# danieleschmidt/spin-torque-rl-gym

Measured on AMD Instinct MI355X. Metric: env_steps_per_sec, higher is better.
Workload: dtype f64

## Files before the change

### spin-torque-rl-gym_amd/csrc/stg_physics.hpp

```cpp
#pragma once

#include <hip/hip_runtime.h>
#include <stdint.h>
#include <type_traits>

#include "stg_minstep.hpp"

namespace stg {

enum ClassConst : int {
    C_EX = 0, C_EY, C_EZ,
    C_HK,
    C_MS,
    C_ALPHA,
    C_GEFF,
    C_POL,
    C_MSV,
    C_HS_SIMPLE,
    C_RX, C_RY, C_RZ,
    C_DX, C_DY, C_DZ,
    C_HEX,
    C_BETA, C_BETAP,
    C_GAMMA,
    C_HS_LLGS,
    C_KUV,
    C_EDEMAG,
    C_NX, C_NY, C_NZ,
    C_AREA, C_RP, C_RAP, C_TMR,
    C_REFX, C_REFY, C_REFZ,
    C_RSERIES,
    C_DEVTYPE,
    C_VALID,
    C_SOT_DL, C_SOT_FL,
    C_SIGX, C_SIGY, C_SIGZ,
    C_KU,
    C_VCMA_XI, C_VCMA_TD2,
    C_VCMA_VBD,
    C_MU0MS,
    C_COUNT
};

template <class P>
__host__ __device__ inline void derive_row(const P& p, double gamma, double temperature, double* r) {
#pragma clang fp contract(off)
    const double mu0 = 4 * 3.14159265358979323846 * 1e-7;
    const double en = sqrt((p.easy_axis[0] * p.easy_axis[0] + p.easy_axis[1] * p.easy_axis[1]) + p.easy_axis[2] * p.easy_axis[2]);
    r[C_EX] = p.easy_axis[0] / en; r[C_EY] = p.easy_axis[1] / en; r[C_EZ] = p.easy_axis[2] / en;
    r[C_HK] = (2 * p.ku) / (mu0 * p.ms);
    r[C_MS] = p.ms;
    r[C_ALPHA] = p.damping;
    r[C_GEFF] = gamma / (1 + p.damping * p.damping);
    r[C_POL] = p.polarization;
    r[C_MSV] = p.ms * p.volume;
    r[C_HS_SIMPLE] = sqrt(2 * p.damping * 1.38e-23 * temperature / (mu0 * p.ms * p.volume * gamma));
    r[C_RX] = p.easy_axis[0]; r[C_RY] = p.easy_axis[1]; r[C_RZ] = p.easy_axis[2];
    r[C_DX] = -p.ms * p.demag[0]; r[C_DY] = -p.ms * p.demag[1]; r[C_DZ] = -p.ms * p.demag[2];
    r[C_HEX] = p.a_ex > 0 ? (2 * p.a_ex / (mu0 * p.ms)) * 0.1 : 0.0;
    r[C_BETA] = p.polarization * gamma / (2 * p.ms * p.volume);
    r[C_BETAP] = 0.1 * r[C_BETA];
    r[C_GAMMA] = gamma;
    r[C_HS_LLGS] = sqrt(2 * p.damping * 1.380649e-23 * temperature / (gamma * mu0 * p.ms * p.volume));
    r[C_KUV] = p.ku * p.volume;
    r[C_EDEMAG] = 0.5 * mu0 * (p.ms * p.ms) * p.volume;
    r[C_NX] = p.demag[0]; r[C_NY] = p.demag[1]; r[C_NZ] = p.demag[2];
    r[C_AREA] = p.area; r[C_RP] = p.r_p; r[C_RAP] = p.r_ap;
    r[C_TMR] = (p.r_ap - p.r_p) / p.r_p;
    const double rn = sqrt((p.ref_m[0] * p.ref_m[0] + p.ref_m[1] * p.ref_m[1]) + p.ref_m[2] * p.ref_m[2]);
    r[C_REFX] = p.ref_m[0] / rn; r[C_REFY] = p.ref_m[1] / rn; r[C_REFZ] = p.ref_m[2] / rn;
    r[C_RSERIES] = p.r_series;
    r[C_DEVTYPE] = (double)p.dev_type;
    r[C_VALID] = p.params_valid ? 1.0 : 0.0;
    r[C_SOT_DL] = p.sot_tau_dl; r[C_SOT_FL] = p.sot_tau_fl;
    r[C_SIGX] = p.sot_sigma[0]; r[C_SIGY] = p.sot_sigma[1]; r[C_SIGZ] = p.sot_sigma[2];
    r[C_KU] = p.ku;
    r[C_VCMA_XI] = p.vcma_xi;
    r[C_VCMA_TD2] = p.vcma_td * p.vcma_td;
    r[C_VCMA_VBD] = p.vcma_vbd;
    r[C_MU0MS] = mu0 * p.ms;
}

struct V3 {
    double x, y, z;
};

__device__ __forceinline__ double mul_x(double a, double b) {
#pragma clang fp contract(off)
    const double r = a * b;
    return r;
}
__device__ __forceinline__ double add_x(double a, double b) {
#pragma clang fp contract(off)
    const double r = a + b;
    return r;
}
__device__ __forceinline__ double sub_x(double a, double b) {
#pragma clang fp contract(off)
    const double r = a - b;
    return r;
}

__device__ __forceinline__ double rsqrt_fast(double s) {
    const double y = __builtin_amdgcn_rsq(s);
    const double e = __builtin_fma(-(s * y), y, 1.0);
    return __builtin_fma(y * e, __builtin_fma(0.375, e, 0.5), y);
}

__device__ __forceinline__ void batch_ready(double at, double a0, double a1, double a2, double b0, double b1, double b2) {
    asm volatile("" : : "v"(at), "v"(a0), "v"(a1), "v"(a2), "v"(b0), "v"(b1), "v"(b2));
}

__device__ __forceinline__ double vgpr_const(double c) {
    asm volatile("" : "+v"(c));
    return c;
}

__device__ __forceinline__ double fmax_abs(double a, double b) {
    double r;
    asm("v_max_f64 %0, |%1|, |%2|" : "=v"(r) : "v"(a), "v"(b));
    return r;
}

__device__ __forceinline__ void commit_step(unsigned long long mask, double& d0, double s0, double& d1, double s1, double& d2, double s2,
                                            double& d3, double s3, double& d4, double s4, double& d5, double s5, double& d6, double s6) {
    unsigned long long saved;
    asm("s_and_saveexec_b64 %[sv], %[m]\n\t"
        "v_mov_b64 %[d0], %[s0]\n\t"
        "v_mov_b64 %[d1], %[s1]\n\t"
        "v_mov_b64 %[d2], %[s2]\n\t"
        "v_mov_b64 %[d3], %[s3]\n\t"
        "v_mov_b64 %[d4], %[s4]\n\t"
        "v_mov_b64 %[d5], %[s5]\n\t"
        "v_mov_b64 %[d6], %[s6]\n\t"
        "s_mov_b64 exec, %[sv]"
        : [d0] "+v"(d0), [d1] "+v"(d1), [d2] "+v"(d2), [d3] "+v"(d3), [d4] "+v"(d4), [d5] "+v"(d5), [d6] "+v"(d6), [sv] "=&s"(saved)
        : [s0] "v"(s0), [s1] "v"(s1), [s2] "v"(s2), [s3] "v"(s3), [s4] "v"(s4), [s5] "v"(s5), [s6] "v"(s6), [m] "s"(mask)
        : "scc");
}

__device__ __forceinline__ double rcp_fast(double x) {
    const double y = __builtin_amdgcn_rcp(x);
    return __builtin_fma(y, __builtin_fma(-x, y, 1.0), y);
}

__device__ __forceinline__ double inv_tenth_root(double e2, double tenth = 0.1) {
    const double y = (double)__builtin_amdgcn_exp2f(-0.1f * __builtin_amdgcn_logf((float)e2));
    const double y2 = y * y, y4 = y2 * y2, y8 = y4 * y4;
    const double e = __builtin_fma(-e2, y8 * y2, 1.0);
    return __builtin_fma(y * e, __builtin_fma(0.055, e, tenth), y);
}

__device__ __forceinline__ double fifth_root(double x) {
    int e;
    const double mant = frexp(x, &e);
    const double t = -0.2 * ((double)e + (double)__builtin_amdgcn_logf((float)mant));
    const double ti = rint(t);
    double r = ldexp((double)__builtin_amdgcn_exp2f((float)(t - ti)), (int)ti);
    const double r2 = r * r, r4 = r2 * r2;
    const double err = __builtin_fma(-x, r4 * r, 1.0);
    r = __builtin_fma(r * err, __builtin_fma(0.12, err, 0.2), r);
    const double q2 = r * r;
    return x * (q2 * q2);
}

__device__ __forceinline__ V3 cross(const V3& a, const V3& b) {
#pragma clang fp contract(off)
    return V3{__builtin_fma(a.y, b.z, -(a.z * b.y)), __builtin_fma(a.z, b.x, -(a.x * b.z)), __builtin_fma(a.x, b.y, -(a.y * b.x))};
}
__device__ __forceinline__ double dot(const V3& a, const V3& b) {
#pragma clang fp contract(off)
    return __builtin_fma(a.z, b.z, __builtin_fma(a.y, b.y, a.x * b.x));
}
__device__ __forceinline__ V3 scale3(double c, const V3& z) {
#pragma clang fp contract(off)
    return V3{c * z.x, c * z.y, c * z.z};
}
__device__ __forceinline__ bool finite3(const V3& a) { return isfinite(a.x) && isfinite(a.y) && isfinite(a.z); }

__device__ __forceinline__ void philox4x32_10(uint32_t c0, uint32_t c1, uint32_t c2, uint32_t c3, uint32_t k0,
                                              uint32_t k1, uint32_t (&out)[4]) {
#pragma unroll
    for (int r = 0; r < 10; ++r) {
        const uint32_t hi0 = __umulhi(0xD2511F53u, c0), lo0 = 0xD2511F53u * c0;
        const uint32_t hi1 = __umulhi(0xCD9E8D57u, c2), lo1 = 0xCD9E8D57u * c2;
        const uint32_t n0 = hi1 ^ c1 ^ k0, n2 = hi0 ^ c3 ^ k1;
        c0 = n0; c1 = lo1; c2 = n2; c3 = lo0;
        k0 += 0x9E3779B9u; k1 += 0xBB67AE85u;
    }
    out[0] = c0; out[1] = c1; out[2] = c2; out[3] = c3;
}

struct NormalStream {
    uint32_t s0, s1, s2, s3;
    float carry;
    __device__ __forceinline__ void init(uint64_t seed, uint64_t env_id, uint32_t env_step, uint32_t tag) {
        uint32_t r[4];
        philox4x32_10((uint32_t)env_id, (uint32_t)(env_id >> 32), env_step, tag, (uint32_t)seed, (uint32_t)(seed >> 32), r);
        s0 = r[0]; s1 = r[1]; s2 = r[2]; s3 = r[3] | 1u;
        carry = 0.0f;
    }
    __device__ __forceinline__ uint32_t next() {
        const uint32_t result = s0 + s3;
        const uint32_t t = s1 << 9;
        s2 ^= s0; s3 ^= s1; s1 ^= s2; s0 ^= s3; s2 ^= t;
        s3 = (s3 << 11) | (s3 >> 21);
        return result;
    }
    __device__ __forceinline__ float uniform() {
        return __uint_as_float(__builtin_amdgcn_alignbit(0x7fu, next(), 9u)) - 0.99999994f;
    }
    typedef float f32x2 __attribute__((ext_vector_type(2)));
    __device__ __forceinline__ void pair(float& a, float& b) {
        float t, c, s_;
        pair_head(t, c, s_);
        finish_pair(t, c, s_, a, b);
    }
    __device__ __forceinline__ void pair_head(float& t, float& c, float& s_) {
        f32x2 u{__uint_as_float(__builtin_amdgcn_alignbit(0x7fu, next(), 9u)), __uint_as_float(__builtin_amdgcn_alignbit(0x7fu, next(), 9u))};
        u = u - f32x2{0.99999994f, 0.99999994f};
        t = -1.3862943611198906f * __builtin_amdgcn_logf(u.x);
        c = __builtin_amdgcn_cosf(u.y);
        s_ = __builtin_amdgcn_sinf(u.y);
    }
    static __device__ __forceinline__ void finish_pair(float t, float c, float s_, float& a, float& b) {
        const float r = __builtin_amdgcn_sqrtf(t);
        const f32x2 cs = f32x2{c, s_} * f32x2{r, r};
        a = cs.x;
        b = cs.y;
    }
    __device__ __forceinline__ V3 draw3_even() {
        float a, b, c, d;
        pair(a, b);
        pair(c, d);
        carry = d;
        return V3{(double)a, (double)b, (double)c};
    }
    __device__ __forceinline__ V3 draw3_odd() {
        float a, b;
        pair(a, b);
        return V3{(double)carry, (double)a, (double)b};
    }
};

struct RngKey {
    uint64_t seed, env_id;
    uint32_t env_step;
};

struct InlineNormals {
    static constexpr bool kShared = false, kScaled = false;
    NormalStream ns;
    __device__ __forceinline__ void begin(const RngKey& rk) { ns.init(rk.seed, rk.env_id, rk.env_step, 0u); }
    __device__ __forceinline__ V3 draw(bool even) { return even ? ns.draw3_even() : ns.draw3_odd(); }
    static constexpr bool broken = false;
    __device__ __forceinline__ void peek() {}
    __device__ __forceinline__ bool chunk_end(bool lane_continues) { return lane_continues; }
    __device__ __forceinline__ bool chunk_end_wave(bool mine) { return mine; }
    __device__ __forceinline__ int32_t chunk_end_go(int32_t go) { return go; }
};

constexpr int SHARED_SUBS_RK4 = 2;
constexpr int SHARED_SUBS3 = 4 * SHARED_SUBS_RK4;
constexpr int SHARED_CHUNK_FIXED = 12 * SHARED_SUBS_RK4;
constexpr int SHARED_CHUNK_RK45 = 18;
constexpr int PC_STOP = 1 << 30;
constexpr int PC_SPIN_CAP = 1 << 22;

typedef __attribute__((address_space(3))) int lds_int;
__device__ __forceinline__ volatile lds_int* lds_flag(const int* p) { return (volatile lds_int*)p; }

template <int WGW>
__device__ __forceinline__ bool any_flag(volatile lds_int* f) {
    int v = f[0];
#pragma unroll
    for (int j = 1; j < WGW; ++j) v |= f[j];
    return v != 0;
}
__device__ __forceinline__ int pc_load(const int* p) {
    return __builtin_amdgcn_readfirstlane(__hip_atomic_load(p, __ATOMIC_ACQUIRE, __HIP_MEMORY_SCOPE_WORKGROUP));
}
__device__ __forceinline__ void pc_store(int* p, int v) {
    __hip_atomic_store(p, v, __ATOMIC_RELEASE, __HIP_MEMORY_SCOPE_WORKGROUP);
}

template <typename T, bool SCALED, int DEPTH, bool BARRIER>
struct SharedNormalsT {
    static constexpr int CHUNK = SCALED ? SHARED_CHUNK_RK45 : SHARED_CHUNK_FIXED;
    static_assert(!BARRIER || DEPTH == 2, "the barrier form runs the producer exactly one chunk ahead");
    static constexpr bool kShared = true, kScaled = SCALED;
    const T* buf;
    int* hs;
    int lane, it, idx, seen;
    bool broken;
    static constexpr bool kToggle = BARRIER && SCALED;
    int slot_b, flag_b;
    __device__ __forceinline__ void begin(const RngKey&) {
        it = 0; idx = 0; seen = 1; broken = false;
        if (kToggle) {
            static_assert(((CHUNK * 64) & 63) == 0, "the slot bit and the lane bits are disjoint");
            slot_b = lane * (int)sizeof(T); flag_b = 0;
            asm volatile("" : "+v"(slot_b), "+v"(flag_b));
        }
    }
    __device__ __forceinline__ V3 draw(bool) {
        const T* b = kToggle ? (const T*)((const char*)buf + slot_b) + idx * 64 : buf + ((it & (DEPTH - 1)) * CHUNK + idx) * 64 + lane;
        idx += 3;
        return V3{(double)b[0], (double)b[64], (double)b[128]};
    }
    __device__ __forceinline__ void peek() {
        if (!BARRIER) seen = __hip_atomic_load(hs, __ATOMIC_RELAXED, __HIP_MEMORY_SCOPE_WORKGROUP);
    }
    __device__ __forceinline__ bool chunk_end(bool lane_continues) { return chunk_end_wave(__ballot(lane_continues) != 0ull); }
    __device__ __forceinline__ bool chunk_end_wave(bool mine) { return chunk_end_go(mine ? 1 : 0) != 0; }
    __device__ __forceinline__ int32_t chunk_end_go(int32_t go) {
        const bool mine = go != 0;
        if (BARRIER) {
            if (kToggle) {
                *(volatile lds_int*)((volatile __attribute__((address_space(3))) char*)lds_flag(hs) + flag_b) = go;
                flag_b ^= (int)sizeof(int); slot_b ^= CHUNK * 64 * (int)sizeof(T);
            } else {
                lds_flag(hs)[it & 1] = go;
            }
            __syncthreads();
            ++it;
            idx = 0;
            return go;
        }
        ++it;
        idx = 0;
        pc_store(hs + 1, it | (mine ? 0 : PC_STOP));
        int have = __builtin_amdgcn_readfirstlane(seen);
        if (__builtin_expect(mine && have <= it, 0)) {
            int spins = 0;
#pragma unroll 1
            do {
                if (spins) __builtin_amdgcn_s_sleep(1);
                have = pc_load(hs);
            } while (have <= it && ++spins <= PC_SPIN_CAP);
            broken = broken || have <= it;
        }
        seen = have;
        __builtin_amdgcn_fence(__ATOMIC_ACQUIRE, "workgroup");
        return (mine && !broken) ? 1 : 0;
    }
};

template <typename T, bool SCALED, int DEPTH, bool BARRIER>
__device__ __forceinline__ void produce_normals(T* buf, int* hs, int lane, const RngKey& rk, int n_first, int n_chunk, double c) {
    NormalStream ns;
    ns.init(rk.seed, rk.env_id, rk.env_step, 0u);
    bool even = true;
    auto fill = [&](int slot, int count) {
        T* b = buf + (slot * (SCALED ? SHARED_CHUNK_RK45 : SHARED_CHUNK_FIXED)) * 64 + lane;
        for (int j = 0; j < count; j += 3) {
            V3 z = even ? ns.draw3_even() : ns.draw3_odd();
            if (SCALED) z = scale3(c, z);
            even = !even;
            b[(j + 0) * 64] = (T)z.x; b[(j + 1) * 64] = (T)z.y; b[(j + 2) * 64] = (T)z.z;
        }
    };
    fill(0, n_first);
    if (!BARRIER) pc_store(hs, 1);
    __syncthreads();
    if (BARRIER) {
        for (int k = 1;; ++k) {
            fill(k & 1, n_chunk);
            __syncthreads();
            if (lds_flag(hs)[(k - 1) & 1] == 0) return;
        }
    }
    for (int k = 1;; ++k) {
        int v = pc_load(hs + 1);
#pragma unroll 1
        for (int spins = 0; (v & (PC_STOP - 1)) < k - DEPTH + 1 && !(v & PC_STOP); ++spins) {
            if (spins > PC_SPIN_CAP) return;
            __builtin_amdgcn_s_sleep(1);
            v = pc_load(hs + 1);
        }
        if (v & PC_STOP) return;
        fill(k & (DEPTH - 1), n_chunk);
        pc_store(hs, k + 1);
    }
}

struct SimpleK {
    V3 e;
    double ghk;
    double gdm;
    double alpha;
    double ghs;
};
__device__ __forceinline__ SimpleK make_simple(const V3& e, double hk, double ms, double alpha, double geff, double hs) {
#pragma clang fp contract(off)
    return SimpleK{e, -geff * hk, geff * ms, alpha, -geff * hs};
}
struct LlgsK {
    V3 r;
    V3 gd;
    double ghk, ghex;
    double alpha;
    double ghs;
    double gz;
    double agz;
};
__device__ __forceinline__ LlgsK make_llgs(const V3& r, const V3& d, double hk, double hex, double alpha, double gamma, double hs) {
#pragma clang fp contract(off)
    const double ng = -gamma;
    const double gz = ng * ((hk * r.z) * r.z + d.z);
    return LlgsK{r, V3{ng * d.x, ng * d.y, ng * d.z}, ng * hk, ng * hex, alpha, ng * hs, gz, alpha * gz};
}


template <bool THERMAL, bool AXIS_Z>
__device__ __forceinline__ V3 simple_rhs(const V3& m, const SimpleK& k, double ghk, double aJ, const V3& z) {
#pragma clang fp contract(off)
    if (AXIS_Z) {
        const double gz = (ghk + k.gdm) * m.z;
        V3 p;
        if (THERMAL) {
            const V3 g{k.ghs * z.x, k.ghs * z.y, __builtin_fma(k.ghs, z.z, gz)};
            p = cross(m, g);
        } else {
            p = V3{m.y * gz, -(m.x * gz), 0.0};
        }
        const double wx = __builtin_fma(k.alpha, p.x, aJ * m.y), wy = __builtin_fma(k.alpha, p.y, -(aJ * m.x));
        if (THERMAL) {
            const double wz = k.alpha * p.z;
            return V3{__builtin_fma(m.y, wz, __builtin_fma(-m.z, wy, p.x)), __builtin_fma(m.z, wx, __builtin_fma(-m.x, wz, p.y)),
                      __builtin_fma(m.x, wy, __builtin_fma(-m.y, wx, p.z))};
        }
        return V3{__builtin_fma(-m.z, wy, p.x), __builtin_fma(m.z, wx, p.y), __builtin_fma(m.x, wy, -(m.y * wx))};
    }
    const V3 t = cross(m, k.e);
    const double c = ghk * dot(m, k.e);
    const double d = k.gdm * m.z;
    V3 p;
    if (THERMAL) {
        const V3 g{__builtin_fma(k.ghs, z.x, c * k.e.x), __builtin_fma(k.ghs, z.y, c * k.e.y),
                   __builtin_fma(k.ghs, z.z, __builtin_fma(c, k.e.z, d))};
        p = cross(m, g);
    } else {
        p = V3{__builtin_fma(c, t.x, d * m.y), __builtin_fma(c, t.y, -(d * m.x)), c * t.z};
    }
    const V3 w{__builtin_fma(k.alpha, p.x, aJ * t.x), __builtin_fma(k.alpha, p.y, aJ * t.y),
               __builtin_fma(k.alpha, p.z, aJ * t.z)};
    return V3{__builtin_fma(m.y, w.z, __builtin_fma(-m.z, w.y, p.x)), __builtin_fma(m.z, w.x, __builtin_fma(-m.x, w.z, p.y)),
              __builtin_fma(m.x, w.y, __builtin_fma(-m.y, w.x, p.z))};
}

struct DevTorque {
    double sdl, sfl;
    V3 sigma;
    double ghk_pulse;
    bool any_sot;
};

__device__ __forceinline__ double vcma_keff(double volt, double ku, double xi, double td2, double vbd) {
    const double v = volt < -vbd ? -vbd : (volt > vbd ? vbd : volt);
    const double keff = ku + (-xi * fabs(v) / td2);
    return fmax(keff, -0.5 * ku);
}

template <bool THERMAL, bool AXIS_Z, bool DEVPHYS>
__device__ __forceinline__ V3 simple_stage(const V3& m, const SimpleK& k, double aJ, const V3& z, const DevTorque& dv,
                                           bool on) {
#pragma clang fp contract(off)
    if (!DEVPHYS) return simple_rhs<THERMAL, AXIS_Z>(m, k, k.ghk, aJ, z);
    V3 f = simple_rhs<THERMAL, AXIS_Z>(m, k, on ? dv.ghk_pulse : k.ghk, aJ, z);
    if (dv.any_sot) {
        const double a = on ? dv.sdl : 0.0, b = on ? dv.sfl : 0.0;
        const V3 sxm = cross(dv.sigma, m);
        f = V3{f.x + __builtin_fma(a, sxm.x, b * dv.sigma.x), f.y + __builtin_fma(a, sxm.y, b * dv.sigma.y),
               f.z + __builtin_fma(a, sxm.z, b * dv.sigma.z)};
    }
    return f;
}

__device__ __forceinline__ int simple_validate(V3& m, bool& zero_row) {
#pragma clang fp contract(off)
    zero_row = false;
    const double e = __builtin_fma(m.z, m.z, __builtin_fma(m.y, m.y, __builtin_fma(m.x, m.x, -1.0)));
    const bool near1 = fabs(e) < 0.0009765625;
    const double inv1 = __builtin_fma(e, __builtin_fma(e, __builtin_fma(e, __builtin_fma(e, 0.2734375, -0.3125), 0.375), -0.5), 1.0);
    if (__builtin_expect(__ballot(!near1) == 0ull, 1)) {
        m = V3{m.x * inv1, m.y * inv1, m.z * inv1};
        return 0;
    }
    const double s = dot(m, m);
    const double inv = near1 ? inv1 : rsqrt_fast(s);
    const bool ordinary = (s >= 1e-24) && (s <= 1.7976931348623157e308);
    if (__builtin_expect(__ballot(!ordinary) == 0ull, 1)) {
        m = V3{m.x * inv, m.y * inv, m.z * inv};
        return 0;
    }
    if (!finite3(m) || s < 1e-24) { m = V3{0.0, 0.0, 1.0}; return 1; }
    m = V3{m.x * inv, m.y * inv, m.z * inv};
    zero_row = isinf(s);
    return 0;
}

__device__ __forceinline__ bool validation_rejects(const V3& m) {
    return !finite3(m) || sqrt(dot(m, m)) < 1e-12;
}

struct SolveOut {
    V3 m;
    int32_t n;
    int32_t resets;
    int64_t work;
    bool ok;
};

struct Recorder {
    double* t;
    double* m;
    double* e;
    double* tq;
    int64_t N, i;
    int32_t cap;
    __device__ __forceinline__ void put(int32_t row, double tt, const V3& mm, double ee, double tqv = 0.0) const {
        if (row < cap) {
            if (t) t[(int64_t)row * N + i] = tt;
            if (m) {
                double* b = m + (int64_t)row * 3 * N + i;
                b[0] = mm.x; b[N] = mm.y; b[2 * N] = mm.z;
            }
            if (e) e[(int64_t)row * N + i] = ee;
            if (tq) tq[(int64_t)row * N + i] = tqv;
        }
    }
};

template <int METHOD, bool THERMAL, bool RECORD, bool AXIS_Z, bool DEVPHYS, class NSRC>
__device__ __forceinline__ SolveOut simple_solve(const V3& m0, double J, double T, const SimpleK& k, double pol,
                                                 double msv, bool class_valid, double temperature, double max_step,
                                                 const RngKey& rk, const Recorder& rec, const DevTorque& dv, NSRC& ns,
                                                 double inv_tau, bool enabled) {
#pragma clang fp contract(off)
    SolveOut o{m0, 0, 0, 0, false};
    const bool rejected_in = !enabled || validation_rejects(m0) || !(T > 0.0) || !class_valid || !(temperature > 0.0);
    if (!NSRC::kShared && rejected_in) return o;
    V3 m = m0;
    bool zr;
    int resets = simple_validate(m, zr);
    double dt = fmin(max_step, (T / 100.0));
    int n = (int)(T / dt);
    n = n < 10 ? 10 : n;
    dt = T / (double)n;
    if (NSRC::kShared && rejected_in) n = 0;
    o.n = n;
    o.work = n;
    const double half_dt = 0.5 * dt, sixth_dt = dt / 6.0;
    const bool useJ = fabs(J) > 1e-12;
    const double aJ = useJ ? (pol * J) / msv : 0.0;
    const double kJ = aJ;
    const double t_last = mul_x((double)(n - 1), dt);
    const bool on2_last = add_x(t_last, mul_x(dt, 0.5)) <= T, on4_last = add_x(t_last, dt) <= T;
    const double kJ2_last = on2_last ? kJ : 0.0;
    const double kJ4_last = on4_last ? kJ : 0.0;
    bool fail = false;
    const V3 zero{0.0, 0.0, 0.0};
    if (THERMAL) ns.begin(rk);
    const bool ou_sel = THERMAL && inv_tau > 0.0;
    double ou_d = 0.0, ou_c = 1.0;
    V3 ou_x = zero;
    if (ou_sel) {
        ou_d = exp(-dt * inv_tau);
        ou_c = sqrt(1.0 - ou_d * ou_d);
    }
    if (RECORD) rec.put(0, 0.0, m, 0.0);
    auto run = [&](auto ou_tag) {
    constexpr bool ou = decltype(ou_tag)::value;
    auto substep = [&](int i, auto which_tag) {
        constexpr int WHICH = decltype(which_tag)::value;
        const bool last = WHICH == 2 ? (i == n - 1) : (WHICH == 1);
        const double kJ2 = last ? kJ2_last : kJ, kJ4 = last ? kJ4_last : kJ;
        const bool on2 = !last || on2_last, on4 = !last || on4_last;
        V3 mn;
        if (METHOD == 1) {
            V3 z0 = zero;
            if (THERMAL) z0 = ns.draw((i & 1) == 0);
            if (ou) {
                ou_x = V3{__builtin_fma(ou_d, ou_x.x, ou_c * z0.x), __builtin_fma(ou_d, ou_x.y, ou_c * z0.y),
                          __builtin_fma(ou_d, ou_x.z, ou_c * z0.z)};
                z0 = ou_x;
            }
            const V3 f = simple_stage<THERMAL, AXIS_Z, DEVPHYS>(m, k, kJ, z0, dv, true);
            mn = V3{__builtin_fma(dt, f.x, m.x), __builtin_fma(dt, f.y, m.y), __builtin_fma(dt, f.z, m.z)};
        } else {
            V3 z0 = zero, z1 = zero, z2 = zero, z3 = zero;
            if (ou) {
                const V3 xi = ns.draw((i & 1) == 0);
                ou_x = V3{__builtin_fma(ou_d, ou_x.x, ou_c * xi.x), __builtin_fma(ou_d, ou_x.y, ou_c * xi.y),
                          __builtin_fma(ou_d, ou_x.z, ou_c * xi.z)};
                z0 = ou_x; z1 = ou_x; z2 = ou_x; z3 = ou_x;
            } else if (THERMAL) {
                z0 = ns.draw(true); z1 = ns.draw(false); z2 = ns.draw(true); z3 = ns.draw(false);
            }
            const V3 f1 = simple_stage<THERMAL, AXIS_Z, DEVPHYS>(m, k, kJ, z0, dv, true);
            const V3 y2{__builtin_fma(half_dt, f1.x, m.x), __builtin_fma(half_dt, f1.y, m.y), __builtin_fma(half_dt, f1.z, m.z)};
            const V3 f2 = simple_stage<THERMAL, AXIS_Z, DEVPHYS>(y2, k, kJ2, z1, dv, on2);
            const V3 y3{__builtin_fma(half_dt, f2.x, m.x), __builtin_fma(half_dt, f2.y, m.y), __builtin_fma(half_dt, f2.z, m.z)};
            const V3 f3 = simple_stage<THERMAL, AXIS_Z, DEVPHYS>(y3, k, kJ2, z2, dv, on2);
            if (THERMAL) ns.peek();
            const V3 y4{__builtin_fma(dt, f3.x, m.x), __builtin_fma(dt, f3.y, m.y), __builtin_fma(dt, f3.z, m.z)};
            const V3 f4 = simple_stage<THERMAL, AXIS_Z, DEVPHYS>(y4, k, kJ4, z3, dv, on4);
            mn = V3{__builtin_fma(sixth_dt, __builtin_fma(2.0, f2.x, f1.x) + __builtin_fma(2.0, f3.x, f4.x), m.x),
                    __builtin_fma(sixth_dt, __builtin_fma(2.0, f2.y, f1.y) + __builtin_fma(2.0, f3.y, f4.y), m.y),
                    __builtin_fma(sixth_dt, __builtin_fma(2.0, f2.z, f1.z) + __builtin_fma(2.0, f3.z, f4.z), m.z)};
        }
        resets += simple_validate(mn, zr);
        fail |= zr;
        m = mn;
        if (RECORD) rec.put(i + 1, last ? T : mul_x((double)(i + 1), dt), m, 0.0);
    };
    if (NSRC::kShared) {
        constexpr int SUBS = (METHOD == 1 || ou) ? SHARED_SUBS3 : SHARED_SUBS_RK4;
        for (int i = 0;; ++i) {
            if (i < n) substep(i, std::integral_constant<int, 2>{});
            if (SUBS == 1 || (i & (SUBS - 1)) == SUBS - 1) {
                if (!ns.chunk_end(i + 1 < n)) break;
            }
        }
    } else {
        for (int i = 0; i < n - 1; ++i) substep(i, std::integral_constant<int, 0>{});
        substep(n - 1, std::integral_constant<int, 1>{});
    }
    };
    if (THERMAL && ou_sel) run(std::true_type{}); else run(std::false_type{});
    const bool rejected_shared = NSRC::kShared && rejected_in;
    o.resets = rejected_shared ? 0 : resets;
    if (fail || rejected_shared || ns.broken) return o;
    o.m = m;
    o.ok = true;
    return o;
}

template <bool THERMAL, bool AXIS_Z, bool CHECKED = true>
__device__ __forceinline__ V3 llgs_rhs(const V3& y, const LlgsK& k, double bJ, double bpJ, const V3& ht) {
#pragma clang fp contract(off)
    const double ss = dot(y, y);
    const double inv = rsqrt_fast(ss);
    V3 m{y.x * inv, y.y * inv, y.z * inv};
    if (CHECKED) {
        const bool unit = ss > 1e-24;
        if (__builtin_expect(__ballot(!unit) != 0ull, 0)) m = V3{unit ? m.x : 0.0, unit ? m.y : 0.0, unit ? m.z : 1.0};
    }
    if (AXIS_Z) {
        const double u = __builtin_fma(k.gz, m.z, bpJ);
        const double w = __builtin_fma(k.agz, m.z, bJ);
        if (!THERMAL) {
            const double c = m.z * w;
            return V3{__builtin_fma(m.x, c, m.y * u), __builtin_fma(m.y, c, -(m.x * u)), __builtin_fma(m.z, c, -w)};
        }
        const double uz = ht.z + u;
        const V3 W{k.alpha * ht.x, k.alpha * ht.y, __builtin_fma(k.alpha, ht.z, w)};
        const double s = dot(m, W);
        return V3{__builtin_fma(m.x, s, __builtin_fma(m.y, uz, __builtin_fma(-m.z, ht.y, -W.x))),
                  __builtin_fma(m.y, s, __builtin_fma(m.z, ht.x, __builtin_fma(-m.x, uz, -W.y))),
                  __builtin_fma(m.z, s, __builtin_fma(m.x, ht.y, __builtin_fma(-m.y, ht.x, -W.z)))};
    }
    const double c = k.ghk * dot(m, k.r);
    V3 g{(c * k.r.x + k.gd.x * m.x) + k.ghex * m.x, (c * k.r.y + k.gd.y * m.y) + k.ghex * m.y,
         (c * k.r.z + k.gd.z * m.z) + k.ghex * m.z};
    if (THERMAL) g = V3{g.x + ht.x, g.y + ht.y, g.z + ht.z};
    const V3 U{g.x, g.y, g.z + bpJ};
    const V3 W{k.alpha * g.x, k.alpha * g.y, __builtin_fma(k.alpha, g.z, bJ)};
    const double s = dot(m, W);
    return V3{__builtin_fma(m.x, s, __builtin_fma(m.y, U.z, __builtin_fma(-m.z, U.y, -W.x))),
              __builtin_fma(m.y, s, __builtin_fma(m.z, U.x, __builtin_fma(-m.x, U.z, -W.y))),
              __builtin_fma(m.z, s, __builtin_fma(m.x, U.y, __builtin_fma(-m.y, U.x, -W.z)))};
}

struct LlgsEnergyK {
    double kuv, edemag;
    V3 r, nfac;
};
__device__ __forceinline__ double llgs_energy(const V3& m, const LlgsEnergyK& k) {
    const double ct = dot(m, k.r);
    return -k.kuv * (ct * ct) + k.edemag * (k.nfac.x * (m.x * m.x) + k.nfac.y * (m.y * m.y) + k.nfac.z * (m.z * m.z));
}

__device__ __forceinline__ double llgs_torque_norms(const V3& m, double bJ, double bpJ) {
#pragma clang fp contract(off)
    const V3 mxp{m.y, -m.x, 0.0};
    const V3 mm = cross(m, mxp);
    const V3 a{bJ * mm.x, bJ * mm.y, bJ * mm.z}, b{bpJ * mxp.x, bpJ * mxp.y, bpJ * mxp.z};
    return sqrt((a.x * a.x + a.y * a.y) + a.z * a.z) + sqrt((b.x * b.x + b.y * b.y) + b.z * b.z);
}

__device__ __forceinline__ double rms3(const V3& a) { return sqrt(dot(a, a)) / 1.7320508075688772; }

struct Dp5Tab {
    double A51, A52, A53, A54, A61, A62, A63, A64, A65, E1, E3, E4, E5, E6, E7;
    double B4, third, c09, tenth;
};
__device__ __forceinline__ Dp5Tab make_dp5_tab() {
    Dp5Tab t;
    t.A51 = vgpr_const(19372.0 / 6561); t.A52 = vgpr_const(-25360.0 / 2187); t.A53 = vgpr_const(64448.0 / 6561); t.A54 = vgpr_const(-212.0 / 729);
    t.A61 = vgpr_const(9017.0 / 3168); t.A62 = vgpr_const(-355.0 / 33); t.A63 = vgpr_const(46732.0 / 5247); t.A64 = vgpr_const(49.0 / 176);
    t.A65 = vgpr_const(-5103.0 / 18656);
    t.E1 = vgpr_const(-71.0 / 57600); t.E3 = vgpr_const(71.0 / 16695); t.E4 = vgpr_const(-71.0 / 1920); t.E5 = vgpr_const(17253.0 / 339200);
    t.E6 = vgpr_const(-22.0 / 525); t.E7 = vgpr_const(1.0 / 40);
    t.B4 = vgpr_const(125.0 / 192); t.third = vgpr_const(1.0 / 3.0); t.c09 = vgpr_const(0.9); t.tenth = vgpr_const(0.1);
    return t;
}

struct LlgsLane {
    V3 y, f;
    V3 m0;
    double t, T, h_abs;
    double h_floor;
    double bJ, bpJ;
    int32_t attempts;
    int32_t npts;
    bool idle;
    bool rejected, active;
};

typedef unsigned long long lanemask;
struct LlgsMasks {
    lanemask active, pacc, low;
};
__device__ __forceinline__ bool lane_in(lanemask m) { return __builtin_amdgcn_inverse_ballot_w64(m); }
__device__ __forceinline__ LlgsMasks llgs_masks_open(const LlgsLane& L) {
    return LlgsMasks{__ballot(L.active), __ballot(!L.rejected), __ballot(L.h_abs < L.h_floor)};
}
__device__ __forceinline__ void llgs_masks_close(LlgsLane& L, const LlgsMasks& M) {
    L.active = lane_in(M.active);
    L.rejected = !lane_in(M.pacc);
}

template <bool RECORD>
__device__ __forceinline__ void llgs_lane_emit(LlgsLane& L, V3& out_m, const Recorder& rec, const LlgsEnergyK& ek) {
    const double inv = rsqrt_fast(dot(L.y, L.y));
    out_m = V3{L.y.x * inv, L.y.y * inv, L.y.z * inv};
    if (RECORD) rec.put(L.npts, L.t, out_m, rec.e ? llgs_energy(out_m, ek) : 0.0, rec.tq ? llgs_torque_norms(out_m, L.bJ, L.bpJ) : 0.0);
    ++L.npts;
}

template <bool THERMAL, bool AXIS_Z, bool CHECKED = true>
__device__ __forceinline__ V3 llgs_fun(const LlgsLane& L, const LlgsK& k, const V3& y, const V3& ht, bool on) {
    return llgs_rhs<THERMAL, AXIS_Z, CHECKED>(y, k, on ? L.bJ : 0.0, on ? L.bpJ : 0.0, ht);
}
template <bool THERMAL, class NSRC>
__device__ __forceinline__ V3 llgs_draw(NSRC& ns, const LlgsK& k, bool even) {
    if (!THERMAL) return V3{0.0, 0.0, 0.0};
    return NSRC::kScaled ? ns.draw(even) : scale3(k.ghs, ns.draw(even));
}

template <bool THERMAL, bool RECORD, bool AXIS_Z, class NSRC>
__device__ __forceinline__ void llgs_lane_begin(LlgsLane& L, V3& out_m, const V3& m0, double J, double T, const LlgsK& k, double beta,
                                                double betap, double rtol, double atol, double max_step, const RngKey& rk,
                                                const Recorder& rec, const LlgsEnergyK& ek, NSRC& ns, bool enabled) {
    const bool useJ = !(fabs(J) < 1e-12);
    L.bJ = useJ ? beta * J : 0.0;
    L.bpJ = useJ ? betap * J : 0.0;
    L.m0 = m0;
    L.T = T;
    if (THERMAL) ns.begin(rk);
    const double n0 = rsqrt_fast(dot(m0, m0));
    L.y = V3{m0.x * n0, m0.y * n0, m0.z * n0};
    L.t = 0.0;
    L.npts = 0;
    if (RECORD) llgs_lane_emit<RECORD>(L, out_m, rec, ek); else ++L.npts;
    L.f = llgs_fun<THERMAL, AXIS_Z>(L, k, L.y, llgs_draw<THERMAL>(ns, k, true), true);
    double h_abs;
    {
        const V3& y = L.y;
        const V3& f = L.f;
        const V3 sc{atol + fabs(y.x) * rtol, atol + fabs(y.y) * rtol, atol + fabs(y.z) * rtol};
        const V3 isc{rcp_fast(sc.x), rcp_fast(sc.y), rcp_fast(sc.z)};
        const double d0 = rms3(V3{y.x * isc.x, y.y * isc.y, y.z * isc.z});
        const double d1 = rms3(V3{f.x * isc.x, f.y * isc.y, f.z * isc.z});
        double h0 = (d0 < 1e-5 || d1 < 1e-5) ? 1e-6 : (0.01 * d0) * rcp_fast(d1);
        h0 = fmin(h0, T);
        const V3 y1{y.x + h0 * f.x, y.y + h0 * f.y, y.z + h0 * f.z};
        const V3 f1 = llgs_fun<THERMAL, AXIS_Z>(L, k, y1, llgs_draw<THERMAL>(ns, k, false), true);
        const double d2 = rms3(V3{(f1.x - f.x) * isc.x, (f1.y - f.y) * isc.y, (f1.z - f.z) * isc.z}) * rcp_fast(h0);
        const double h1 = (d1 <= 1e-15 && d2 <= 1e-15) ? fmax(1e-6, h0 * 1e-3) : fifth_root(0.01 * rcp_fast(fmax(d1, d2)));
        h_abs = fmin(fmin(100.0 * h0, h1), fmin(T, max_step));
    }
    L.rejected = false;
    L.attempts = 0;
    const double min_step = min_step_at(L.t);
    L.h_abs = h_abs > max_step ? max_step : (h_abs < min_step ? min_step : h_abs);
    L.h_floor = isfinite(T) ? min_step_at(T) : __builtin_inf();
    L.active = enabled && (L.t != T);
    L.idle = !L.active;
}

template <bool UNIFORM_IT>
__device__ __forceinline__ void llgs_lane_gate(LlgsLane& L, LlgsMasks& M, int32_t max_attempts) {
    if (__builtin_expect((M.low & M.active) != 0ull, 0)) {
        const double min_step = min_step_at(L.t);
        if (lane_in(M.pacc)) L.h_abs = L.h_abs < min_step ? min_step : L.h_abs;
        M.active &= ~__ballot(L.h_abs < min_step);
    }
    if (!UNIFORM_IT) M.active &= ~__ballot(L.attempts >= max_attempts);
}

__device__ __forceinline__ int32_t attempt_loop_next(lanemask& active, lanemask not_arrived, int32_t& it, int32_t budget) {
    int32_t go;
    asm("s_add_i32 %[it], %[it], 1\n\t"
        "s_and_b64 %[act], %[act], %[na]\n\t"
        "s_cselect_b32 %[go], %[bud], 0\n\t"
        "s_cmp_lt_i32 %[it], %[go]\n\t"
        "s_cselect_b32 %[go], 1, 0"
        : [act] "+s"(active), [it] "+s"(it), [go] "=&s"(go)
        : [na] "s"(not_arrived), [bud] "s"(budget)
        : "scc");
    return go;
}

template <bool THERMAL, bool RECORD, bool AXIS_Z, bool UNIFORM_IT, class NSRC>
__device__ __forceinline__ void llgs_lane_attempt(LlgsLane& L, LlgsMasks& M, V3& out_m, const LlgsK& k, const Dp5Tab& tb, double rtol,
                                                  double atol, double max_step, const Recorder& rec, const LlgsEnergyK& ek, NSRC& ns, V3 z2, V3 z3) {
    constexpr double A21 = 1.0 / 5;
    constexpr double A31 = 3.0 / 40, A32 = 9.0 / 40;
    constexpr double A41 = 44.0 / 45, A42 = -56.0 / 15, A43 = 32.0 / 9;
    constexpr double B1 = 35.0 / 384, B3 = 500.0 / 1113, B5 = -2187.0 / 6784, B6 = 11.0 / 84;
    const double B4 = tb.B4;
    const double A51 = tb.A51, A52 = tb.A52, A53 = tb.A53, A54 = tb.A54, A61 = tb.A61, A62 = tb.A62, A63 = tb.A63, A64 = tb.A64, A65 = tb.A65;
    const double E1 = tb.E1, E3 = tb.E3, E4 = tb.E4, E5 = tb.E5, E6 = tb.E6, E7 = tb.E7;
    const double T = L.T;
    const bool active = lane_in(M.active);
    const V3 y = L.y;
    const double t = L.t;
    auto fun = [&](const V3& yy, const V3& ht, bool on) -> V3 { return llgs_fun<THERMAL, AXIS_Z, false>(L, k, yy, ht, on); };
    auto draw = [&](bool even) -> V3 { return llgs_draw<THERMAL>(ns, k, even); };
    L.attempts += active ? 1 : 0;
    const double t_new = fmin(add_x(t, L.h_abs), T);
    const double h = sub_x(t_new, t);
    const double h_try = fabs(h);
    const bool on_end = add_x(t, h) <= T;
    const V3 k1 = L.f;
    constexpr bool BATCH = THERMAL && NSRC::kShared;
    if (THERMAL && !NSRC::kShared) { z2 = draw(true); z3 = draw(false); }
    V3 y2{y.x + (k1.x * A21) * h, y.y + (k1.y * A21) * h, y.z + (k1.z * A21) * h};
    if (BATCH) batch_ready(y2.z, z2.x, z2.y, z2.z, z3.x, z3.y, z3.z);
    const V3 k2 = fun(y2, z2, true);
    V3 z4 = draw(true), z5{0.0, 0.0, 0.0};
    if (BATCH) { z5 = draw(false); __builtin_amdgcn_sched_barrier(0); }
    const V3 k3 = fun(V3{y.x + (k1.x * A31 + k2.x * A32) * h, y.y + (k1.y * A31 + k2.y * A32) * h,
                         y.z + (k1.z * A31 + k2.z * A32) * h}, z3, true);
    if (!BATCH) z5 = draw(false);
    V3 y4{y.x + (k1.x * A41 + k2.x * A42 + k3.x * A43) * h, y.y + (k1.y * A41 + k2.y * A42 + k3.y * A43) * h,
          y.z + (k1.z * A41 + k2.z * A42 + k3.z * A43) * h};
    if (BATCH) batch_ready(y4.z, z4.x, z4.y, z4.z, z5.x, z5.y, z5.z);
    const V3 k4 = fun(y4, z4, true);
    V3 z6 = draw(true), z7{0.0, 0.0, 0.0};
    if (BATCH) { z7 = draw(false); __builtin_amdgcn_sched_barrier(0); }
    const V3 k5 = fun(V3{y.x + (k1.x * A51 + k2.x * A52 + k3.x * A53 + k4.x * A54) * h,
                         y.y + (k1.y * A51 + k2.y * A52 + k3.y * A53 + k4.y * A54) * h,
                         y.z + (k1.z * A51 + k2.z * A52 + k3.z * A53 + k4.z * A54) * h}, z5, true);
    if (THERMAL) ns.peek();
    if (!BATCH) z7 = draw(false);
    V3 y6{y.x + (k1.x * A61 + k2.x * A62 + k3.x * A63 + k4.x * A64 + k5.x * A65) * h,
          y.y + (k1.y * A61 + k2.y * A62 + k3.y * A63 + k4.y * A64 + k5.y * A65) * h,
          y.z + (k1.z * A61 + k2.z * A62 + k3.z * A63 + k4.z * A64 + k5.z * A65) * h};
    if (BATCH) batch_ready(y6.z, z6.x, z6.y, z6.z, z7.x, z7.y, z7.z);
    const V3 k6 = fun(y6, z6, on_end);
    const V3 y_new{y.x + h * (k1.x * B1 + k3.x * B3 + k4.x * B4 + k5.x * B5 + k6.x * B6),
                   y.y + h * (k1.y * B1 + k3.y * B3 + k4.y * B4 + k5.y * B5 + k6.y * B6),
                   y.z + h * (k1.z * B1 + k3.z * B3 + k4.z * B4 + k5.z * B5 + k6.z * B6)};
    const V3 f_new = fun(y_new, z7, on_end);
    const V3 ev{(k1.x * E1 + k3.x * E3 + k4.x * E4 + k5.x * E5 + k6.x * E6 + f_new.x * E7) * h,
                (k1.y * E1 + k3.y * E3 + k4.y * E4 + k5.y * E5 + k6.y * E6 + f_new.y * E7) * h,
                (k1.z * E1 + k3.z * E3 + k4.z * E4 + k5.z * E5 + k6.z * E6 + f_new.z * E7) * h};
    const V3 sc{atol + fmax_abs(y.x, y_new.x) * rtol, atol + fmax_abs(y.y, y_new.y) * rtol, atol + fmax_abs(y.z, y_new.z) * rtol};
    const V3 q{ev.x * rcp_fast(sc.x), ev.y * rcp_fast(sc.y), ev.z * rcp_fast(sc.z)};
    const double err2 = dot(q, q) * tb.third;
    const double err = err2;
    const lanemask accm = M.active & __ballot(err < 1.0);
    const bool acc = lane_in(accm);
    const double r9 = tb.c09 * inv_tenth_root(err, tb.tenth);
    const double fa = fmin(lane_in(M.pacc) ? 10.0 : 1.0, r9);
    const double fr = fmax(0.2, r9);
    double h_next = fmin(h_try * (acc ? fa : fr), max_step);
    M.low = __ballot(h_next < L.h_floor);
    L.h_abs = h_next;
    commit_step(accm, L.t, t_new, L.y.x, y_new.x, L.y.y, y_new.y, L.y.z, y_new.z, L.f.x, f_new.x, L.f.y, f_new.y, L.f.z, f_new.z);
    if (RECORD) { if (acc) llgs_lane_emit<RECORD>(L, out_m, rec, ek); } else L.npts += acc ? 1 : 0;
    M.pacc = accm;
    if (!UNIFORM_IT) M.active &= __ballot(L.t != T);
}

template <bool RECORD, class NSRC>
__device__ __forceinline__ SolveOut llgs_lane_finish(LlgsLane& L, V3& out_m, const Recorder& rec, const LlgsEnergyK& ek, const NSRC& ns) {
    SolveOut o{L.m0, 0, 0, 0, false};
    if (!RECORD) { llgs_lane_emit<RECORD>(L, out_m, rec, ek); --L.npts; }
    o.m = out_m;
    o.n = L.npts - 1;
    o.work = L.attempts;
    const bool ok = L.idle || L.t == L.T;
    o.ok = ok && !ns.broken;
    if (!ok) o.m = L.m0;
    return o;
}

template <bool THERMAL, bool RECORD, bool AXIS_Z, class NSRC>
__device__ __forceinline__ SolveOut llgs_solve(const V3& m0, double J, double T, const LlgsK& k, double beta,
                                               double betap, double rtol, double atol, double max_step,
                                               int64_t max_attempts, const RngKey& rk, const Recorder& rec,
                                               const LlgsEnergyK& ek, NSRC& ns, bool enabled) {
    const Dp5Tab tb = make_dp5_tab();
    const V3 zero{0.0, 0.0, 0.0};
    LlgsLane L;
    V3 out_m = m0;
    llgs_lane_begin<THERMAL, RECORD, AXIS_Z>(L, out_m, m0, J, T, k, beta, betap, rtol, atol, max_step, rk, rec, ek, ns, enabled);
    LlgsMasks M = llgs_masks_open(L);
    atol = vgpr_const(atol);
    int32_t budget = (int32_t)max_attempts;
    asm volatile("" : "+s"(budget));
    int32_t it = 0;
    bool wave_go = M.active != 0ull;
    if (NSRC::kShared) wave_go = ns.chunk_end_wave(wave_go);
    if (wave_go)
    for (;;) {
      V3 z2 = zero, z3 = zero;
      if (THERMAL && NSRC::kShared) { z2 = llgs_draw<THERMAL>(ns, k, true); z3 = llgs_draw<THERMAL>(ns, k, false); }
      llgs_lane_gate<true>(L, M, budget);
      llgs_lane_attempt<THERMAL, RECORD, AXIS_Z, true>(L, M, out_m, k, tb, rtol, atol, max_step, rec, ek, ns, z2, z3);
      if (!ns.chunk_end_go(attempt_loop_next(M.active, __ballot(L.t != L.T), it, budget))) break;
    }
    llgs_masks_close(L, M);
    return llgs_lane_finish<RECORD>(L, out_m, rec, ek, ns);
}

__device__ __forceinline__ double resistance(const V3& m_in, int dev_type, double r_p, double r_ap, double tmr,
                                             const V3& ref, double r_series) {
#pragma clang fp contract(off)
    if (dev_type == 0) {
        const double inv = rsqrt_fast(dot(m_in, m_in));
        const V3 m{m_in.x * inv, m_in.y * inv, m_in.z * inv};
        const double r = r_p * (1.0 + tmr * (1.0 - dot(m, ref)) * 0.5);
        return fmax(r, r_p * 0.5);
    }
    double r = r_p + (r_ap - r_p) * (1.0 - dot(m_in, ref)) * 0.5;
    if (dev_type == 1) r = r + r_series;
    return fmax(r, 1.0);
}

template <typename AT>
__device__ __forceinline__ void parse_action(AT a0, AT a1, double max_current, double max_duration, double& J, double& T) {
    const AT cmax = (AT)1e8, dmin = (AT)1e-12, dmax = (AT)1e-6;
    if (!isnan(a0)) a0 = a0 < -cmax ? -cmax : (a0 > cmax ? cmax : a0);
    if (!isnan(a1)) a1 = a1 < dmin ? dmin : (a1 > dmax ? dmax : a1);
    if (isnan(a0) || isnan(a1) || isinf(a0) || isinf(a1)) { a0 = (AT)0; a1 = dmin; }
    const double j = (double)a0, t = (double)a1;
    J = j < -max_current ? -max_current : (j > max_current ? max_current : j);
    T = t < 1e-12 ? 1e-12 : (t > max_duration ? max_duration : t);
}

__device__ __forceinline__ float obs_cast(double v) {
    const float f = (float)v;
    return isnan(f) ? 0.0f : (isinf(f) ? (f > 0 ? 1e6f : -1e6f) : f);
}

}
```

Measured before the change: 44.16 million.

## Split chunk-end sync into publish/rendezvous and overlap with step-size refinement

Splits the shared-noise chunk-end handshake into a publish step (write the LDS flag) and a rendezvous step (barrier or spin). The publish moves inside the RK45 attempt, right after the step commit, so the loop-continue decision is posted before the step-size controller's tenth-root refinement runs. The inverse tenth-root is split into a seed and a refine stage so the transcendental seed can issue early. A hook in the RHS pins where the batched noise operands are ready, with added sched_barriers to fix scheduling. The aim is to hide barrier latency behind arithmetic; the cost is tighter scheduling constraints that may block other compiler reordering.

```diff
diff --git a/spin-torque-rl-gym_amd/csrc/stg_physics.hpp b/spin-torque-rl-gym_amd/csrc/stg_physics.hpp
--- a/spin-torque-rl-gym_amd/csrc/stg_physics.hpp
+++ b/spin-torque-rl-gym_amd/csrc/stg_physics.hpp
@@ -109,6 +109,11 @@
     asm volatile("" : : "v"(at), "v"(a0), "v"(a1), "v"(a2), "v"(b0), "v"(b1), "v"(b2));
 }
 
+struct NoHook {
+    template <class... A>
+    __device__ __forceinline__ void operator()(A&&...) const {}
+};
+
 __device__ __forceinline__ double vgpr_const(double c) {
     asm volatile("" : "+v"(c));
     return c;
@@ -142,11 +147,16 @@
     return __builtin_fma(y, __builtin_fma(-x, y, 1.0), y);
 }
 
-__device__ __forceinline__ double inv_tenth_root(double e2, double tenth = 0.1) {
-    const double y = (double)__builtin_amdgcn_exp2f(-0.1f * __builtin_amdgcn_logf((float)e2));
+__device__ __forceinline__ double inv_tenth_root_seed(double e2) {
+    return (double)__builtin_amdgcn_exp2f(-0.1f * __builtin_amdgcn_logf((float)e2));
+}
+__device__ __forceinline__ double inv_tenth_root_refine(double e2, double y, double tenth) {
     const double y2 = y * y, y4 = y2 * y2, y8 = y4 * y4;
     const double e = __builtin_fma(-e2, y8 * y2, 1.0);
     return __builtin_fma(y * e, __builtin_fma(0.055, e, tenth), y);
+}
+__device__ __forceinline__ double inv_tenth_root(double e2, double tenth = 0.1) {
+    return inv_tenth_root_refine(e2, inv_tenth_root_seed(e2), tenth);
 }
 
 __device__ __forceinline__ double fifth_root(double x) {
@@ -256,6 +266,8 @@
     __device__ __forceinline__ bool chunk_end(bool lane_continues) { return lane_continues; }
     __device__ __forceinline__ bool chunk_end_wave(bool mine) { return mine; }
     __device__ __forceinline__ int32_t chunk_end_go(int32_t go) { return go; }
+    __device__ __forceinline__ void publish(int32_t) {}
+    __device__ __forceinline__ int32_t rendezvous(int32_t go) { return go; }
 };
 
 constexpr int SHARED_SUBS_RK4 = 2;
@@ -312,14 +324,18 @@
     __device__ __forceinline__ bool chunk_end(bool lane_continues) { return chunk_end_wave(__ballot(lane_continues) != 0ull); }
     __device__ __forceinline__ bool chunk_end_wave(bool mine) { return chunk_end_go(mine ? 1 : 0) != 0; }
     __device__ __forceinline__ int32_t chunk_end_go(int32_t go) {
+        publish(go);
+        return rendezvous(go);
+    }
+    __device__ __forceinline__ void publish(int32_t go) {
+        if (!BARRIER) return;
+        if (kToggle) *(volatile lds_int*)((volatile __attribute__((address_space(3))) char*)lds_flag(hs) + flag_b) = go;
+        else lds_flag(hs)[it & 1] = go;
+    }
+    __device__ __forceinline__ int32_t rendezvous(int32_t go) {
         const bool mine = go != 0;
         if (BARRIER) {
-            if (kToggle) {
-                *(volatile lds_int*)((volatile __attribute__((address_space(3))) char*)lds_flag(hs) + flag_b) = go;
-                flag_b ^= (int)sizeof(int); slot_b ^= CHUNK * 64 * (int)sizeof(T);
-            } else {
-                lds_flag(hs)[it & 1] = go;
-            }
+            if (kToggle) { flag_b ^= (int)sizeof(int); slot_b ^= CHUNK * 64 * (int)sizeof(T); }
             __syncthreads();
             ++it;
             idx = 0;
@@ -635,8 +651,8 @@
     return o;
 }
 
-template <bool THERMAL, bool AXIS_Z, bool CHECKED = true>
-__device__ __forceinline__ V3 llgs_rhs(const V3& y, const LlgsK& k, double bJ, double bpJ, const V3& ht) {
+template <bool THERMAL, bool AXIS_Z, bool CHECKED = true, class MID = NoHook>
+__device__ __forceinline__ V3 llgs_rhs(const V3& y, const LlgsK& k, double bJ, double bpJ, const V3& ht, MID mid = MID{}) {
 #pragma clang fp contract(off)
     const double ss = dot(y, y);
     const double inv = rsqrt_fast(ss);
@@ -652,6 +668,7 @@
             const double c = m.z * w;
             return V3{__builtin_fma(m.x, c, m.y * u), __builtin_fma(m.y, c, -(m.x * u)), __builtin_fma(m.z, c, -w)};
         }
+        mid(w);
         const double uz = ht.z + u;
         const V3 W{k.alpha * ht.x, k.alpha * ht.y, __builtin_fma(k.alpha, ht.z, w)};
         const double s = dot(m, W);
@@ -662,7 +679,7 @@
     const double c = k.ghk * dot(m, k.r);
     V3 g{(c * k.r.x + k.gd.x * m.x) + k.ghex * m.x, (c * k.r.y + k.gd.y * m.y) + k.ghex * m.y,
          (c * k.r.z + k.gd.z * m.z) + k.ghex * m.z};
-    if (THERMAL) g = V3{g.x + ht.x, g.y + ht.y, g.z + ht.z};
+    if (THERMAL) { mid(g.z); g = V3{g.x + ht.x, g.y + ht.y, g.z + ht.z}; }
     const V3 U{g.x, g.y, g.z + bpJ};
     const V3 W{k.alpha * g.x, k.alpha * g.y, __builtin_fma(k.alpha, g.z, bJ)};
     const double s = dot(m, W);
@@ -738,9 +755,9 @@
     ++L.npts;
 }
 
-template <bool THERMAL, bool AXIS_Z, bool CHECKED = true>
-__device__ __forceinline__ V3 llgs_fun(const LlgsLane& L, const LlgsK& k, const V3& y, const V3& ht, bool on) {
-    return llgs_rhs<THERMAL, AXIS_Z, CHECKED>(y, k, on ? L.bJ : 0.0, on ? L.bpJ : 0.0, ht);
+template <bool THERMAL, bool AXIS_Z, bool CHECKED = true, class MID = NoHook>
+__device__ __forceinline__ V3 llgs_fun(const LlgsLane& L, const LlgsK& k, const V3& y, const V3& ht, bool on, MID mid = MID{}) {
+    return llgs_rhs<THERMAL, AXIS_Z, CHECKED>(y, k, on ? L.bJ : 0.0, on ? L.bpJ : 0.0, ht, mid);
 }
 template <bool THERMAL, class NSRC>
 __device__ __forceinline__ V3 llgs_draw(NSRC& ns, const LlgsK& k, bool even) {
@@ -812,9 +829,10 @@
     return go;
 }
 
-template <bool THERMAL, bool RECORD, bool AXIS_Z, bool UNIFORM_IT, class NSRC>
+template <bool THERMAL, bool RECORD, bool AXIS_Z, bool UNIFORM_IT, class NSRC, class HOOK = NoHook>
 __device__ __forceinline__ void llgs_lane_attempt(LlgsLane& L, LlgsMasks& M, V3& out_m, const LlgsK& k, const Dp5Tab& tb, double rtol,
-                                                  double atol, double max_step, const Recorder& rec, const LlgsEnergyK& ek, NSRC& ns, V3 z2, V3 z3) {
+                                                  double atol, double max_step, const Recorder& rec, const LlgsEnergyK& ek, NSRC& ns, V3 z2, V3 z3,
+                                                  HOOK committed = HOOK{}) {
     constexpr double A21 = 1.0 / 5;
     constexpr double A31 = 3.0 / 40, A32 = 9.0 / 40;
     constexpr double A41 = 44.0 / 45, A42 = -56.0 / 15, A43 = 32.0 / 9;
@@ -837,8 +855,9 @@
     constexpr bool BATCH = THERMAL && NSRC::kShared;
     if (THERMAL && !NSRC::kShared) { z2 = draw(true); z3 = draw(false); }
     V3 y2{y.x + (k1.x * A21) * h, y.y + (k1.y * A21) * h, y.z + (k1.z * A21) * h};
-    if (BATCH) batch_ready(y2.z, z2.x, z2.y, z2.z, z3.x, z3.y, z3.z);
-    const V3 k2 = fun(y2, z2, true);
+    const V3 k2 = llgs_fun<THERMAL, AXIS_Z, false>(L, k, y2, z2, true, [&](double at) {
+        if (BATCH) { batch_ready(at, z2.x, z2.y, z2.z, z3.x, z3.y, z3.z); __builtin_amdgcn_sched_barrier(0); }
+    });
     V3 z4 = draw(true), z5{0.0, 0.0, 0.0};
     if (BATCH) { z5 = draw(false); __builtin_amdgcn_sched_barrier(0); }
     const V3 k3 = fun(V3{y.x + (k1.x * A31 + k2.x * A32) * h, y.y + (k1.y * A31 + k2.y * A32) * h,
@@ -858,7 +877,7 @@
     V3 y6{y.x + (k1.x * A61 + k2.x * A62 + k3.x * A63 + k4.x * A64 + k5.x * A65) * h,
           y.y + (k1.y * A61 + k2.y * A62 + k3.y * A63 + k4.y * A64 + k5.y * A65) * h,
           y.z + (k1.z * A61 + k2.z * A62 + k3.z * A63 + k4.z * A64 + k5.z * A65) * h};
-    if (BATCH) batch_ready(y6.z, z6.x, z6.y, z6.z, z7.x, z7.y, z7.z);
+    if (BATCH) { batch_ready(y6.z, z6.x, z6.y, z6.z, z7.x, z7.y, z7.z); __builtin_amdgcn_sched_barrier(0); }
     const V3 k6 = fun(y6, z6, on_end);
     const V3 y_new{y.x + h * (k1.x * B1 + k3.x * B3 + k4.x * B4 + k5.x * B5 + k6.x * B6),
                    y.y + h * (k1.y * B1 + k3.y * B3 + k4.y * B4 + k5.y * B5 + k6.y * B6),
@@ -873,14 +892,16 @@
     const double err = err2;
     const lanemask accm = M.active & __ballot(err < 1.0);
     const bool acc = lane_in(accm);
-    const double r9 = tb.c09 * inv_tenth_root(err, tb.tenth);
+    const double seed = inv_tenth_root_seed(err);
+    commit_step(accm, L.t, t_new, L.y.x, y_new.x, L.y.y, y_new.y, L.y.z, y_new.z, L.f.x, f_new.x, L.f.y, f_new.y, L.f.z, f_new.z);
+    if (RECORD) { if (acc) llgs_lane_emit<RECORD>(L, out_m, rec, ek); } else L.npts += acc ? 1 : 0;
+    committed();
+    const double r9 = tb.c09 * inv_tenth_root_refine(err, seed, tb.tenth);
     const double fa = fmin(lane_in(M.pacc) ? 10.0 : 1.0, r9);
     const double fr = fmax(0.2, r9);
     double h_next = fmin(h_try * (acc ? fa : fr), max_step);
     M.low = __ballot(h_next < L.h_floor);
     L.h_abs = h_next;
-    commit_step(accm, L.t, t_new, L.y.x, y_new.x, L.y.y, y_new.y, L.y.z, y_new.z, L.f.x, f_new.x, L.f.y, f_new.y, L.f.z, f_new.z);
-    if (RECORD) { if (acc) llgs_lane_emit<RECORD>(L, out_m, rec, ek); } else L.npts += acc ? 1 : 0;
     M.pacc = accm;
     if (!UNIFORM_IT) M.active &= __ballot(L.t != T);
 }
@@ -920,6 +941,17 @@
       V3 z2 = zero, z3 = zero;
       if (THERMAL && NSRC::kShared) { z2 = llgs_draw<THERMAL>(ns, k, true); z3 = llgs_draw<THERMAL>(ns, k, false); }
       llgs_lane_gate<true>(L, M, budget);
+      if (NSRC::kShared) {
+          int32_t go = 0;
+          llgs_lane_attempt<THERMAL, RECORD, AXIS_Z, true>(L, M, out_m, k, tb, rtol, atol, max_step, rec, ek, ns, z2, z3, [&]() {
+              go = attempt_loop_next(M.active, __ballot(L.t != L.T), it, budget);
+              ns.publish(go);
+              __builtin_amdgcn_sched_barrier(0);
+          });
+          __builtin_amdgcn_sched_barrier(0);
+          if (!ns.rendezvous(go)) break;
+          continue;
+      }
       llgs_lane_attempt<THERMAL, RECORD, AXIS_Z, true>(L, M, out_m, k, tb, rtol, atol, max_step, rec, ek, ns, z2, z3);
       if (!ns.chunk_end_go(attempt_loop_next(M.active, __ballot(L.t != L.T), it, budget))) break;
     }
```

After: 44.34 million (median of 6 runs). About the same (+0.4%).
